# calavera/patrol

Hardware: AMD Instinct MI355X
Metric: bucket-state merges/sec + achieved HBM GB/s at 1/2/4/8 MI355X (higher is better)
Workload: dtype f64; 1 GPU; C2 merge: 100000000 replica messages -> 10000000-bucket table (2^25 slots), Zipf(1.1); keys_per_gpu=10000000, slots_per_gpu=33554432, parallelism=shard1, name_bytes=2-8 (b<id>), world_size=1, full=False, exchange=False, batches_in_hbm=28

## Files before the change

### patrol_amd/csrc/phip_engine.hip

```cpp
#include <sys/random.h>

#include <chrono>
#include <cstdlib>
#include <cstring>
#include <hip/hip_runtime.h>
#include <rocprim/rocprim.hpp>

#include <algorithm>
#include <cstdarg>
#include <cstdio>
#include <cstring>
#include <mutex>
#include <string>
#include <vector>

#include "patrolhip.h"
#include "phip_kernels.hpp"
#include "phip_host.hpp"

using namespace phip;

namespace {

#ifndef PHIP_SORT_BITS
// ... 617 lines not shown
  out->cap = shard_cap(units, per_unit);
  if ((rc = ensure(h, base_id, (size_t)kShards * out->cap, &out->base)) ||
      (rc = ensure(h, B_MSCNT, 2 * kShards, &out->cnt)))
    return rc;
  if (zero) HIPCHK(h, hipMemsetAsync(out->cnt, 0, kShards * sizeof(u32), h->stream));
  return PHIP_OK;
}

int pack_sharded(phip_handle* h, const Sharded& sh, u32 total_slot, u32* out, u32* total) {
  k_shard_scan<<<1, kShards, 0, h->stream>>>(sh.cnt, h->ctr, total_slot, nullptr, 0, nullptr,
                                             nullptr, nullptr);
  HIPCHK(h, hipGetLastError());
  int rc;
  if ((rc = read_ctr(h))) return rc;
  *total = h->ctr_host[total_slot];
  if (*total) {
    Launch l(h, "k_shard_compact");
    dim3 grid(grid_for(h->ctr_host[kCtrShardMax]), kShards);
    k_shard_compact<<<grid, 256, 0, h->stream>>>(sh.base, sh.cap, sh.cnt, out);
    HIPCHK(h, hipGetLastError());
  }
  return PHIP_OK;
}


enum class PassAsk { kPolicy, kMayUndo, kIsolate, kNoIsolate };

template <class In>
PassKind pass_kind(const phip_handle* h, PassAsk ask) {
  if (ask == PassAsk::kIsolate) return PassKind::kIsolating;
  if (ask == PassAsk::kNoIsolate) return PassKind::kClassified;
  if (h->iso_always || h->iso_left > 0) return PassKind::kIsolating;
  if (ask == PassAsk::kMayUndo && In::kSoa && !h->classify_first && h->opt_left == 0)
    return PassKind::kOptimistic;
  return PassKind::kClassified;
}

inline size_t undo_counts(const phip_handle* h) { return (size_t)h->ncu * kFastPerCU * (kFastBlock / 64); }

struct UndoLayout {
  u32 grid, waves, cap;
  u64 halves;
};
inline UndoLayout undo_layout(u32 n, u32 ncu) {
  UndoLayout l;
  l.grid = fast_grid_on(ncu, n);
  l.waves = l.grid * (kFastBlock / 64);
  l.cap = undo_wave_cap(n, l.grid);
  l.halves = (u64)l.waves * l.cap * 2;
  return l;
}

inline u32* fctr(phip_handle* h, u32 par) { return h->ctr + kCtrWords * (1 + par); }

inline u32* fast_counts(phip_handle* h, u32 par) {
  return (u32*)h->buf[B_FSCNT].p + par * 2 * kShards;
}

int dirty_set(phip_handle* h, DirtySet* d, u32** dlist) {
  int rc;
  u64* b;
  if ((rc = ensure(h, B_DTAB, DirtySet::kWords, &b)) || (rc = ensure(h, B_DLIST, kDirtyCap, dlist)))
    return rc;
  *d = DirtySet::at(b);
  return PHIP_OK;
}
struct SubBatch {
  uint64_t *off, *a, *t;
  int64_t* e;
  u8* len;
  u32* map;
};
int sub_batch(phip_handle* h, SubBatch* b) {
  constexpr size_t m = kSubBatchCap;
  int rc;
  if ((rc = ensure(h, B_SOFF, m, &b->off)) || (rc = ensure(h, B_SLEN, m, &b->len)) ||
      (rc = ensure(h, B_SA, m, &b->a)) || (rc = ensure(h, B_ST, m, &b->t)) ||
      (rc = ensure(h, B_SE, m, &b->e)) || (rc = ensure(h, B_SMAP, m, &b->map)))
    return rc;
  return PHIP_OK;
}

int fast_shards(phip_handle* h, u32 n, u32 par, Sharded* out) {
  int rc;
  u32* c;
  out->cap = shard_cap((n + 63) / 64, 64);
  if ((rc = ensure(h, B_MSHARD, (size_t)kShards * out->cap, &out->base)) ||
      (rc = ensure(h, B_FSCNT, 4 * kShards, &c)))
    return rc;
  out->cnt = fast_counts(h, par);
  return PHIP_OK;
}

template <class Src>
int fork_hot(phip_handle* h, Src src, FastPass* p) {
  if (p->n < kHotMinBatch) return PHIP_OK;
  HIPCHK(h, hipStreamWaitEvent(h->stream2, h->ev_fork, 0));
  int rc;
  if ((rc = build_hot(h, src, p->n, h->stream2, nullptr, p))) return rc;
  HIPCHK(h, hipEventRecord(h->ev_join, h->stream2));
  p->hot_join = true;
  return PHIP_OK;
}

bool keep_take(phip_handle* h, FastPass* p);
template <class HotSrc>
// ... 63 lines not shown
  p->c = fctr(h, p->par);
  ++h->nfast;
  if (reset) {
    k_batch_reset<<<1, kShards, 0, h->stream>>>(p->c, fast_counts(h, p->par));
    HIPCHK(h, hipGetLastError());
  }
  if (p->kind == PassKind::kOptimistic) return front_optimistic(h, hsrc, status, p);
  h->keep.agree = false;
  return front_classified(h, in, hsrc, status, p);
}

inline bool holds(const phip_handle* h, BufId id, size_t bytes) {
  return h->buf[id].cap >= std::max<size_t>(bytes, 64) + 64;
}
inline bool back_fits(const phip_handle* h, u32 n) {
  return holds(h, B_MISS, (size_t)n * sizeof(u32)) &&
         holds(h, B_MSHARD, (size_t)kShards * shard_cap((n + 63) / 64, 64) * sizeof(u32)) &&
         holds(h, B_FSCNT, 4 * kShards * sizeof(u32)) &&
         holds(h, B_ULOG, (size_t)undo_layout(n, (u32)h->ncu).halves * sizeof(u64x2));
}

template <class In>
int fast_back(phip_handle* h, In in, FastPass& p, bool queued) {
  const u32 n = p.n;
  const bool iso = p.kind == PassKind::kIsolating;
  u32* miss;
  int rc;
  Sharded msh;
  DirtySet dset{};
  SubBatch sb{};
  u32* dlist = nullptr;
  if ((rc = ensure(h, B_MISS, n, &miss)) || (rc = fast_shards(h, n, p.par, &msh))) return rc;
  if (iso) {
    if ((rc = dirty_set(h, &dset, &dlist)) || (rc = sub_batch(h, &sb))) return rc;
    Launch l(h, "k_dirty_build");
    k_dirty_build<In><<<1, 1024, 0, h->stream>>>(in, n, p.c, dlist, dset, table(h));
    HIPCHK(h, hipGetLastError());
  }
  if (p.hot_join) HIPCHK(h, hipStreamWaitEvent(h->stream, h->ev_join, 0));
  switch (p.kind) {
    case PassKind::kOptimistic:
      if constexpr (In::kSoa) {
        const UndoLayout ul = undo_layout(n, (u32)h->ncu);
        p.log.cap = ul.cap;
        if ((rc = ensure(h, B_ULOG, (size_t)ul.halves, &p.log.base))) return rc;
        u8* kstatus = PHIP_STATUS_IN_KERNEL ? p.fill : nullptr;
        if (p.fill && !kstatus) HIPCHK(h, hipMemsetAsync(p.fill, PHIP_ST_MERGED, n, h->stream));
        Launch l(h, "k_receive_fast");
        auto* kern = p.hot_nw == 2   ? k_receive_fast<In, true, 2>
                     : p.hot_nw == 3 ? k_receive_fast<In, true, 3>
                                     : k_receive_fast<In, true, 0>;
        kern<<<ul.grid, kFastBlock, 0, h->stream>>>(
            in, 0, n, table(h), msh, p.c, p.hot, p.dir, nullptr, nullptr, p.log,
            (uint4*)p.hot_zero, p.hot_age != 0, p.gate, kstatus);
      }
      break;
    case PassKind::kClassified:
    case PassKind::kIsolating: {
      Launch l(h, "k_receive_fast");
      k_receive_fast<In><<<fast_grid(h, n), kFastBlock, 0, h->stream>>>(
          in, 0, n, table(h), msh, p.c, p.hot, p.dir, iso ? dset.key : nullptr, p.mark,
          UndoLog{}, (uint4*)p.hot_zero, 0u, nullptr, nullptr);
    }
  }
  HIPCHK(h, hipGetLastError());
  if (p.hot_zero) h->hot_clean = p.hot_zero;
  if (iso) {
    {
      Launch l(h, "k_dirty_pass");
      const unsigned g = (unsigned)std::max<u64>(
          1, std::min<u64>(((u64)n + 1023) / 1024, (u64)h->ncu * 2));
      k_dirty_pass<In><<<g, 1024, 0, h->stream>>>(in, n, p.c, p.mark, dset.key, table(h), msh);
      HIPCHK(h, hipGetLastError());
    }
    k_batch_end<In><<<1, kShards, 0, h->stream>>>(
        in, p.c, dset.key, table(h),
        SubOut{sb.off, sb.len, sb.a, sb.t, sb.e, sb.map, kSubBatchCap}, msh.cnt,
        h->ctr_map + kCtrWords * (1 + p.par), kCtrWords,
        queued ? fast_counts(h, p.par ^ 1u) : nullptr, fctr(h, p.par ^ 1u));
  } else {
    k_shard_scan<<<1, kShards, 0, h->stream>>>(msh.cnt, p.c, kCtrMiss,
                                               h->ctr_map + kCtrWords * (1 + p.par), kCtrWords,
                                               queued ? fast_counts(h, p.par ^ 1u) : nullptr,
                                               fctr(h, p.par ^ 1u), p.gate);
  }
  HIPCHK(h, hipGetLastError());
  HIPCHK(h, hipEventRecord(h->ev_ctr[p.par], h->stream));
  if (!queued) HIPCHK(h, hipEventSynchronize(h->ev_ctr[p.par]));
  return PHIP_OK;
}

constexpr u32 kIsoKeep = 256;
constexpr u32 kOptBackoff = 256;

constexpr u32 kHotKeepPasses = 32;
bool keep_take(phip_handle* h, FastPass* p) {
  phip_handle::HotKeep& k = h->keep;
  if (p->n < kHotMinBatch || !k.have || !k.agree || k.sagged || k.served >= kHotKeepPasses ||
      k.gen != h->layout_gen || k.base != h->buf[B_HOT].p)
    return false;
  p->hot = (const HotHdr*)((u8*)k.base + kHotSlotsAt + k.slot * kHotSlotBytes);
  p->dir = (const HotEntry*)(p->hot + 1);
  p->hot_age = k.served++;
  p->hot_nw = k.maxlen <= kShortName ? 2u : k.maxlen <= kInlineName ? 3u : 0u;
  return true;
}
bool keep_sagged(const phip_handle* h, const FastPass& p, const u32* c) {
  const phip_handle::HotKeep& k = h->keep;
  return p.hot_age != 0 && (unsigned __int128)c[kCtrHotHits] * k.ref_n * 8 <
                               (unsigned __int128)k.ref_hits * p.n * 7;
}
void keep_collect(phip_handle* h, const FastPass& p, const u32* c) {
  phip_handle::HotKeep& k = h->keep;
  if (p.kind != PassKind::kOptimistic) {
    k.agree = false;
    return;
  }
  if (p.built) {
    k.agree = c[kCtrHotOwn] > 0 && (u64)c[kCtrHotKept] * 8 >= (u64)c[kCtrHotOwn] * 7;
    k.maxlen = c[kCtrHotMaxLen];
    k.ref_hits = c[kCtrHotHits];
    k.ref_n = p.n;
    k.sagged = false;
  } else if (keep_sagged(h, p, c)) {
    k.sagged = true;
  }
}

inline const u32* fmirror(const phip_handle* h, u32 par) { return h->ctr_host + kCtrWords * (1 + par); }

bool apply_policy(phip_handle* h, const FastPass& p) {
  const u32* c = fmirror(h, p.par);
  if (p.kind == PassKind::kOptimistic) {
// ... 1348 lines not shown
  *out = nullptr;
  if (cfg->log2_slots < 4 || cfg->log2_slots > 31) return PHIP_ERR_INVALID;
  int ndev = 0;
  if (hipGetDeviceCount(&ndev) != hipSuccess || ndev == 0) return PHIP_ERR_NO_DEVICE;
  if (cfg->device < 0 || cfg->device >= ndev) return PHIP_ERR_NO_DEVICE;
  phip_handle* h = new phip_handle;
  h->device = cfg->device;
  h->L = h->L_open = cfg->log2_slots;
  h->cap = 1ull << h->L;
  h->load_pct = cfg->max_load_pct ? std::min<u32>(cfg->max_load_pct, 95) : 90;
  h->max_load = load_limit(h->cap, h->load_pct);
  h->grow = !(cfg->flags & PHIP_CFG_NO_GROW);
  h->iso_always = cfg->flags & PHIP_CFG_ISOLATE;
  h->classify_first = cfg->flags & PHIP_CFG_CLASSIFY_FIRST;
  h->small = !(cfg->flags & PHIP_CFG_NO_SMALL);
  h->track = cfg->flags & PHIP_CFG_TRACK_CHANGES;
  h->arena_cap = h->arena_open = cfg->arena_bytes ? cfg->arena_bytes : (1ull << 20);
  if (cfg->debug_tag_bits && cfg->debug_tag_bits < 64) h->tag_mask = (1ull << cfg->debug_tag_bits) - 1;
  if (cfg->flags & PHIP_CFG_FIXED_SEED) {
    h->seed = cfg->hash_seed;
  } else if (getrandom(&h->seed, sizeof h->seed, 0) != (ssize_t)sizeof h->seed) {
    h->seed = seeded_mix((u64)std::chrono::steady_clock::now().time_since_epoch().count(),
                         (u64)(uintptr_t)h);
  }
  auto fail = [&](hipError_t e) {
    phip_close(h);
    (void)e;
    return PHIP_ERR_HIP;
  };
  hipError_t e;
  if ((e = hipSetDevice(h->device)) != hipSuccess) return fail(e);
  if ((e = hipDeviceGetAttribute(&h->ncu, hipDeviceAttributeMultiprocessorCount, h->device)) !=
      hipSuccess)
    return fail(e);
  if ((e = hipStreamCreateWithFlags(&h->own_stream, hipStreamNonBlocking)) != hipSuccess)
    return fail(e);
  h->stream = h->own_stream;
  if ((e = hipStreamCreateWithFlags(&h->stream2, hipStreamNonBlocking)) != hipSuccess) return fail(e);
  if ((e = hipStreamCreateWithFlags(&h->stream3, hipStreamNonBlocking)) != hipSuccess) return fail(e);
  if ((e = hipEventCreateWithFlags(&h->ev_fork, hipEventDisableTiming)) != hipSuccess) return fail(e);
  if ((e = hipEventCreateWithFlags(&h->ev_join, hipEventDisableTiming)) != hipSuccess) return fail(e);
  if ((e = hipEventCreateWithFlags(&h->ev_fork3, hipEventDisableTiming)) != hipSuccess) return fail(e);
  if ((e = hipEventCreateWithFlags(&h->ev_join3, hipEventDisableTiming)) != hipSuccess) return fail(e);
  if ((e = hipEventCreateWithFlags(&h->ev_gather, hipEventDisableTiming)) != hipSuccess) return fail(e);
  if ((e = hipEventCreateWithFlags(&h->ev_gather3, hipEventDisableTiming)) != hipSuccess)
    return fail(e);
  if ((e = hipEventCreateWithFlags(&h->ev_pack, hipEventDisableTiming)) != hipSuccess) return fail(e);
  for (hipEvent_t& ev : h->ev_ctr)
    if ((e = hipEventCreateWithFlags(&ev, hipEventDisableTiming)) != hipSuccess) return fail(e);
  if ((e = hipMalloc(&h->recs, h->cap * sizeof(Rec))) != hipSuccess) return fail(e);
  if ((e = hipMalloc(&h->aux, h->cap * sizeof(u32))) != hipSuccess) return fail(e);
  if ((e = hipMalloc(&h->arena, h->arena_cap + 64)) != hipSuccess) return fail(e);
  if ((e = hipMalloc(&h->arena_cursor, 64)) != hipSuccess) return fail(e);
  if ((e = hipMalloc(&h->ctr, 3 * kCtrWords * sizeof(u32))) != hipSuccess) return fail(e);
  if ((e = hipHostMalloc(&h->ctr_host, 3 * kCtrWords * sizeof(u32),
                         hipHostMallocMapped | hipHostMallocCoherent)) != hipSuccess ||
      (e = hipHostGetDevicePointer((void**)&h->ctr_map, h->ctr_host, 0)) != hipSuccess)
    return fail(e);
  if ((e = hipMemsetAsync(h->recs, 0, h->cap * sizeof(Rec), h->stream)) != hipSuccess) return fail(e);
  if ((e = hipMemsetAsync(h->aux, 0, h->cap * sizeof(u32), h->stream)) != hipSuccess) return fail(e);
  if (h->track && alloc_marks(h, h->cap, &h->marks)) return fail(hipErrorOutOfMemory);
  if ((e = hipMemsetAsync(h->arena_cursor, 0, 64, h->stream)) != hipSuccess) return fail(e);
  if ((e = hipMemsetAsync(h->ctr, 0, 3 * kCtrWords * sizeof(u32), h->stream)) != hipSuccess)
    return fail(e);
  if ((e = hipStreamSynchronize(h->stream)) != hipSuccess) return fail(e);
  *out = h;
  return PHIP_OK;
}

void phip_close(phip_handle* h) {
  if (!h) return;
  (void)hipSetDevice(h->device);
  if (h->pend.active) (void)after_error(h, finish_pending(h));
  if (h->stream) (void)hipStreamSynchronize(h->stream);
  if (h->stream2) (void)hipStreamSynchronize(h->stream2);
  if (h->stream3) (void)hipStreamSynchronize(h->stream3);
  if (h->stream4) (void)hipStreamSynchronize(h->stream4);
  for (auto& b : h->buf)
    if (b.p) (void)hipFree(b.p);
  for (auto& t : h->event_pool) {
    (void)hipEventDestroy(t.a);
    (void)hipEventDestroy(t.b);
  }
  if (h->recs) (void)hipFree(h->recs);
  if (h->aux) (void)hipFree(h->aux);
  if (h->marks.state) (void)hipFree(h->marks.state);
  if (h->arena) (void)hipFree(h->arena);
  if (h->arena_cursor) (void)hipFree(h->arena_cursor);
  if (h->ctr) (void)hipFree(h->ctr);
  if (h->ctr_host) (void)hipHostFree(h->ctr_host);
  if (h->small_pin) (void)hipHostFree(h->small_pin);
  if (h->ev_fork) (void)hipEventDestroy(h->ev_fork);
  if (h->ev_join) (void)hipEventDestroy(h->ev_join);
  if (h->ev_fork3) (void)hipEventDestroy(h->ev_fork3);
  if (h->ev_join3) (void)hipEventDestroy(h->ev_join3);
  if (h->ev_gather) (void)hipEventDestroy(h->ev_gather);
  if (h->ev_gather3) (void)hipEventDestroy(h->ev_gather3);
  if (h->ev_pack) (void)hipEventDestroy(h->ev_pack);
  for (hipEvent_t ev : h->ev_ctr)
    if (ev) (void)hipEventDestroy(ev);
  if (h->stream2) (void)hipStreamDestroy(h->stream2);
  if (h->stream3) (void)hipStreamDestroy(h->stream3);
  if (h->stream4) (void)hipStreamDestroy(h->stream4);
  if (h->ev_t4a) (void)hipEventDestroy(h->ev_t4a);
  if (h->ev_t4b) (void)hipEventDestroy(h->ev_t4b);
  if (h->own_stream) {
    (void)hipStreamSynchronize(h->own_stream);
    (void)hipStreamDestroy(h->own_stream);
  }
  delete h;
}

const char* phip_last_error(const phip_handle* h) { return h ? h->err.c_str() : "null handle"; }

int phip_flush(phip_handle* h) {
  if (!h) return PHIP_ERR_INVALID;
// ... 1908 lines not shown
```

### patrol_amd/csrc/phip_kernels.hpp

```cpp
#pragma once
#include <type_traits>

#include "phip_device.hpp"

namespace phip {

constexpr int kBlock = 256;

template <bool NT, class T>
__device__ inline T ld(const T* p) {
  if constexpr (NT) return __builtin_nontemporal_load(p);
  else return *p;
}

__device__ inline u64 load_be64(const u8* p) {
  u64 v = 0;
#pragma unroll
  for (int k = 0; k < 8; ++k) v = (v << 8) | p[k];
  return v;
}

struct NamesOffs {
  const u8* blob;
  const u32* offs;
// ... 173 lines not shown
constexpr u32 kCtrHotExt = 23;
constexpr u32 kCtrHotMaxLen = 24;
constexpr u32 kCtrGateShut = 22;
constexpr u32 kCtrEgIncast = kCtrHotExt;
constexpr u32 kCtrEgN = kCtrHotMaxLen;
constexpr u32 kCtrEgErr = 25;
constexpr u32 kCtrEgIncastBytes = 26;
constexpr u32 kCtrEgBytes = 28;
constexpr u32 kCtrChgMarks = 30;
constexpr u32 kCtrChgCleared = 31;
constexpr u32 kCtrWords = 32;
__host__ __device__ constexpr u32 ctr_reset_value(u32 w) {
  return (w == kCtrStop || w == kCtrDirty) ? ~0u : 0u;
}
static_assert(kCtrNDirty < kCtrResetWords && kCtrBadName < kCtrResetWords &&
                  kCtrOccupied < kCtrResetWords && kCtrStop < kCtrResetWords &&
                  kCtrLogOver < kCtrResetWords && kCtrLogCount < kCtrResetWords &&
                  kCtrArenaFull < kCtrResetWords && kCtrTableFull < kCtrResetWords &&
                  kCtrHotHits < kCtrResetWords && kCtrDirty < kCtrResetWords,
              "the words kernels accumulate into from the batch's reset value");
static_assert(kCtrTableFull == kCtrArenaFull + 1, "evict_idle clears both flags in one memset");
static_assert(kCtrLongBytes % 2 == 0 && kCtrLongBytes >= kCtrResetWords &&
              kCtrLongBytes + 2 <= kCtrWords, "an aligned u64 outside the reset");
static_assert(kCtrNDefer >= kCtrResetWords && kCtrNDefer < kCtrWords &&
              kCtrNSorted >= kCtrResetWords && kCtrNSorted < kCtrWords &&
              kCtrHotOwn >= kCtrResetWords && kCtrHotKept < kCtrWords &&
              kCtrGateShut >= kCtrResetWords && kCtrGateShut < kCtrWords, "outside the reset");
static_assert(kCtrEgIncast > kCtrGateShut && kCtrEgErr < kCtrEgIncastBytes &&
              kCtrEgIncastBytes % 2 == 0 && kCtrEgBytes == kCtrEgIncastBytes + 2 &&
              kCtrEgBytes + 2 <= kCtrWords, "the egress words: two aligned u64 behind three u32");
static_assert(kCtrChgMarks == kCtrEgBytes + 2 && kCtrChgCleared == kCtrChgMarks + 1 &&
              kCtrChgCleared < kCtrWords, "the change set's words: zeroed in one memset");

__host__ __device__ inline bool gate_shut(const u32* c) {
  return c[kCtrDirty] != ~0u || c[kCtrStop] != ~0u || c[kCtrNDirty] != 0 || c[kCtrLogOver] != 0 ||
         c[kCtrMiss] != 0 || c[kCtrTableFull] != 0;
}
static_assert(kCtrResetWords <= kShards && kCtrWords <= kShards,
              "k_batch_reset and shard_scan's host mirror: one lane per word");

__global__ __launch_bounds__(kShards) void k_batch_reset(u32* ctr, u32* shard_cnt) {
  const u32 t = threadIdx.x;
  if (t < kCtrResetWords) ctr[t] = ctr_reset_value(t);
  if (shard_cnt) shard_cnt[t] = 0;
}

__device__ inline void shard_scan(u32* cnt, u32* ctr, u32 tot, u32* host, u32 words, u32* next,
                                  u32* next_ctr, const u32* gate = nullptr);
__global__ __launch_bounds__(kShards) void k_shard_scan(u32* cnt, u32* ctr, u32 tot, u32* host,
                                                        u32 words, u32* next, u32* next_ctr,
                                                        const u32* gate) {
  shard_scan(cnt, ctr, tot, host, words, next, next_ctr, gate);
}
__device__ inline void shard_scan(u32* cnt, u32* ctr, u32 tot, u32* host, u32 words, u32* next,
                                  u32* next_ctr, const u32* gate) {
  __shared__ u32 v[kShards];
  __shared__ u32 wmax[kShards / 64];
  if (gate && gate_shut(gate)) next = nullptr;
  const u32 t = threadIdx.x, c = cnt[t];
  v[t] = c;
  u32 m = c;
  for (u32 d = 32; d; d >>= 1) m = max(m, (u32)__shfl_xor((int)m, d));
  if ((t & 63) == 0) wmax[t >> 6] = m;
  __syncthreads();
  for (u32 off = 1; off < kShards; off <<= 1) {
    const u32 x = t >= off ? v[t - off] : 0u;
    __syncthreads();
    v[t] += x;
    __syncthreads();
  }
  cnt[kShards + t] = v[t] - c;
  const u32 total = v[kShards - 1];
  u32 mx = 0;
  for (u32 w = 0; w < kShards / 64; ++w) mx = max(mx, wmax[w]);
  if (t == 0) {
    ctr[tot] = total;
    ctr[kCtrShardMax] = mx;
  }
  if (host && t < words) {
    const u32 w = t == tot ? total : t == kCtrShardMax ? mx : ctr[t];
    __hip_atomic_store(&host[t], w, __ATOMIC_RELAXED, __HIP_MEMORY_SCOPE_SYSTEM);
  }
  if (next) {
    if (t < kCtrResetWords) next_ctr[t] = ctr_reset_value(t);
    next[t] = 0;
  }
}

__global__ __launch_bounds__(256) void k_shard_compact(const u32* __restrict__ base, u32 cap,
                                                       const u32* __restrict__ cnt,
                                                       u32* __restrict__ out) {
  const u32 s = blockIdx.y, j = blockIdx.x * 256 + threadIdx.x;
  if (j < cnt[s]) out[cnt[kShards + s] + j] = base[(size_t)s * cap + j];
}

template <bool Co = false>
__device__ inline bool name_equal(const Rec& r, const Name& nm, const u8* src, const u8* arena) {
  const u64 r0 = r.name0 & ~0xFF00ull;
  if ((r0 & 0xFFu) != (nm.w0 & 0xFFu)) return false;
  if (nm.len <= kInlineName) return r0 == nm.w0 && r.name1 == nm.w1 && r.name2 == nm.w2;
  if (r.name1 != nm.w1 || r.name2 != nm.w2) return false;
  return long_tail_equal<Co>(arena, r.name0 >> 32, src, nm.off, nm.len);
}

enum ProbeResult : int { kFound = 0, kMiss = 1, kPending = 2, kFull = 3 };

__host__ __device__ inline u64 seeded_mix(u64 tag, u64 seed) {
  u64 x = tag ^ seed;
  x ^= x >> 33;
  x *= 0xff51afd7ed558ccdull;
  x ^= x >> 33;
  x *= 0xc4ceb9fe1a85ec53ull;
  x ^= x >> 33;
  return x;
}

struct Table {
  Rec* recs;
  u32* aux;
  const u8* arena;
  u32 L;
  u64 tag_mask;
  u64 seed;
  __device__ inline u64 tag(u64 h) const { return tag_of(h & tag_mask); }
  __device__ inline u32 home(u64 tag) const { return (u32)(seeded_mix(tag, seed) >> (64 - L)); }
  __device__ inline u32 mask() const { return (u32)((1ull << L) - 1); }
};

__device__ inline Rec load_rec(const Rec* p) {
  const uint4* q = reinterpret_cast<const uint4*>(p);
  uint4 a = q[0], b = q[1], c = q[2], d = q[3];
  Rec r;
  r.tag = ((u64)a.y << 32) | a.x;
  r.added = ((u64)a.w << 32) | a.z;
  r.taken = ((u64)b.y << 32) | b.x;
  r.elapsed = (i64)(((u64)b.w << 32) | b.z);
  r.name0 = ((u64)c.y << 32) | c.x;
  r.name1 = ((u64)c.w << 32) | c.z;
  r.created = (i64)(((u64)d.y << 32) | d.x);
// ... 883 lines not shown
  return eq;
}

constexpr u8 kMarkDirty = 0x40;

#ifndef PHIP_UNDO_NT
#define PHIP_UNDO_NT 1
#endif
#ifndef PHIP_STATUS_IN_KERNEL
#define PHIP_STATUS_IN_KERNEL 1
#endif
constexpr u32 kUndoFlushReserve = 64 * ((kHotMax + kFastBlock - 1) / kFastBlock);
struct UndoLog {
  u64x2* base = nullptr;
  u32* cnt = nullptr;
  u32 cap = 0;
};
__host__ __device__ inline u32 fast_wave_chunks(u32 n, u32 grid) {
  const u32 nchunks = (n + 63) / 64, kw = kFastBlock / 64;
  if (grid % 8 == 0) {
    const u32 per = (nchunks + 7) / 8, waves = grid / 8 * kw;
    return (per + waves - 1) / waves;
  }
  return (nchunks + grid * kw - 1) / (grid * kw);
}
constexpr u32 kUndoSlack = 24;
__host__ __device__ inline u32 undo_wave_cap(u32 n, u32 grid) {
  return fast_wave_chunks(n, grid) * 32 + kUndoSlack + kUndoFlushReserve;
}
__device__ inline u32 lane_rank(u64 m) {
  return __builtin_amdgcn_mbcnt_hi((u32)(m >> 32), __builtin_amdgcn_mbcnt_lo((u32)m, 0u));
}
__device__ inline void undo_store(u64x2* p, u32 slot, u64 a, u64 t, i64 e) {
#if PHIP_UNDO_NT
  __builtin_nontemporal_store(u64x2{(u64)slot, a}, p);
  __builtin_nontemporal_store(u64x2{t, (u64)e}, p + 1);
#else
  p[0] = u64x2{(u64)slot, a};
  p[1] = u64x2{t, (u64)e};
#endif
}

template <u32 NW>
struct HotCompact {
  static constexpr u32 kMax = NW == 2 ? kHotMaxExt : kHotMax3;
  static constexpr u32 kNameMax = NW == 2 ? kShortName : kInlineName;
  u16 hidx[kHotIdx];
  u64 hw[NW][kMax];
  u64 hmax[3][kMax];
  u32 hrec[kMax];
};
static_assert(sizeof(HotCompact<2>) == hot_compact_bytes(2, kHotMaxExt) &&
              sizeof(HotCompact<3>) == hot_compact_bytes(3, kHotMax3), "the layouts' arithmetic");
template <class In, bool Opt = false, u32 NW = 0>
__global__ __launch_bounds__(kFastBlock) __attribute__((amdgpu_waves_per_eu(8, 8))) void k_receive_fast(
    In in, u32 lo, u32 n, Table T, Sharded miss, u32* ctr,
    const HotHdr* __restrict__ hot, const HotEntry* __restrict__ hot_dir, const u64* dtab,
    u8* __restrict__ mark, UndoLog ulog, uint4* __restrict__ hot_zero, u32 hot_kept,
    const u32* gate, u8* __restrict__ status) {
  if constexpr (Opt) {
    const bool shut = gate && gate_shut(gate);
    if (blockIdx.x == 0 && threadIdx.x == 0) ctr[kCtrGateShut] = shut;
    if (shut) return;
    if (PHIP_STATUS_IN_KERNEL == 1 && status) {
      constexpr u32 b4 = PHIP_ST_MERGED * 0x01010101u;
      const u64 head = min((u64)n, (u64)(-(uintptr_t)status & 15));
      const u64 n16 = (n - head) / 16;
      uint4* body = reinterpret_cast<uint4*>(status + head);
      for (u64 k = (u64)blockIdx.x * kFastBlock + threadIdx.x; k < n16; k += (u64)gridDim.x * kFastBlock)
        body[k] = uint4{b4, b4, b4, b4};
      if (blockIdx.x == 0) {
        if (threadIdx.x < head) status[threadIdx.x] = PHIP_ST_MERGED;
        const u64 done = head + n16 * 16;
        if (done + threadIdx.x < n) status[done + threadIdx.x] = PHIP_ST_MERGED;
      }
    }
  }
  __shared__ u32 hslot[kHotLds];
  __shared__ u64 htag[kHotMax], hw0[kHotMax], hw1[kHotMax], hw2[kHotMax];
  __shared__ u32 hrec[kHotMax], haoff[kHotMax];
  __shared__ u64 htail[kHotTailWords][kHotMax];
  __shared__ u64 hmax[3][kHotMax];
  static_assert(NW == 0 || (Opt && In::kSoa && (NW == 2 || NW == 3)), "compact: optimistic, decoded");
  using Compact = HotCompact<NW ? NW : 2>;
  __shared__ Compact hc;
  static_assert(NW != 0 || sizeof(hslot) + sizeof(htag) * 4 + sizeof(hrec) * 2 + sizeof(htail) +
                                   sizeof(hmax) + 64 <= kHotLdsBudget,
                "today's layout in half a CU's LDS");
  __shared__ u32 hhits;
  __shared__ u32 hlog[2];

  if (hot_zero)
    for (u32 k = blockIdx.x * kFastBlock + threadIdx.x; k < kHotZeroBytes / sizeof(uint4);
         k += gridDim.x * kFastBlock)
      hot_zero[k] = uint4{0, 0, 0, 0};
  const u32 ndr = !Opt && dtab ? ctr[kCtrNDirty] : 0u;
  const bool iso = !Opt && ndr != 0 && ndr <= kDirtyCap;
  if constexpr (!Opt) n = min(n, iso ? ctr[kCtrStop] : min(ctr[kCtrStop], ctr[kCtrDirty]));
  if (n <= lo) return;
  const u32 nh = !hot ? 0u : NW ? min(hot->n_ext, Compact::kMax) : min(hot->n, kHotMax);
  if constexpr (NW != 0) {
    u32* const hidx32 = reinterpret_cast<u32*>(hc.hidx);
    for (u32 j = threadIdx.x; j < kHotIdx / 2; j += kFastBlock) hidx32[j] = 0;
    for (u32 j = threadIdx.x; j < Compact::kMax; j += kFastBlock) {
      hc.hmax[0][j] = 0; hc.hmax[1][j] = 0; hc.hmax[2][j] = 0;
    }
  } else {
    for (u32 j = threadIdx.x; j < kHotLds; j += kFastBlock) hslot[j] = 0;
    for (u32 j = threadIdx.x; j < kHotMax; j += kFastBlock) {
      hmax[0][j] = 0; hmax[1][j] = 0; hmax[2][j] = 0;
    }
  }
  if (threadIdx.x == 0) hhits = 0;
  if (Opt && threadIdx.x < 2) hlog[threadIdx.x] = 0;
  __syncthreads();
  if constexpr (NW != 0) {
    u32* const hidx32 = reinterpret_cast<u32*>(hc.hidx);
    for (u32 j = threadIdx.x; j < nh; j += kFastBlock) {
      const HotEntry d = hot_dir[j];
      hc.hw[0][j] = d.w0; hc.hw[1][j] = d.w1;
      if constexpr (NW == 3) hc.hw[2][j] = d.w2;
      hc.hrec[j] = d.slot;
      bool same = (u32)(d.w0 & 0xFFu) <= Compact::kNameMax && d.slot <= T.mask();
      if (same) {
        const Rec r = load_rec(&T.recs[d.slot]);
        same = r.tag == d.tag && (rec_flags(r) & kRecPublished) && (r.name0 & ~0xFF00ull) == d.w0 &&
               r.name1 == d.w1 && r.name2 == d.w2;
      }
      if (!same) continue;
      const u32 val = (j + 1) | (hot_fp(d.tag) << 11);
      for (u32 hs = hot_home_idx(d.tag);;) {
        const u32 sh = (hs & 1) * 16;
        const u32 old = __hip_atomic_load(&hidx32[hs >> 1], __ATOMIC_RELAXED, __HIP_MEMORY_SCOPE_WORKGROUP);
        if ((old >> sh) & 0xFFFFu) { hs = (hs + 1) & (kHotIdx - 1); continue; }
        if (atomicCAS(&hidx32[hs >> 1], old, old | (val << sh)) == old) break;
      }
    }
  } else
  for (u32 j = threadIdx.x; j < nh; j += kFastBlock) {
    const HotEntry d = hot_dir[j];
    htag[j] = d.tag; hw0[j] = d.w0; hw1[j] = d.w1; hw2[j] = d.w2;
    hrec[j] = d.slot | (iso && (rec_flags(T.recs[d.slot]) & kRecDirty) ? 0x80000000u : 0u);
    haoff[j] = d.aoff;
    for (u32 k = 0; k < kHotTailWords; ++k) htail[k][j] = d.tail[k];
    if (hot_kept) {
      bool same = d.slot <= T.mask();
      if (same) {
        const Rec r = load_rec(&T.recs[d.slot]);
        const bool arena = (r.name0 & 0xFFu) > kInlineName;
        same = r.tag == d.tag && (rec_flags(r) & kRecPublished) &&
               (arena ? (r.name0 & 0xFFu) : (r.name0 & ~0xFF00ull)) == d.w0 && r.name1 == d.w1 &&
               r.name2 == d.w2 && (arena ? (u32)(r.name0 >> 32) : 0u) == d.aoff;
      }
// ... 142 lines not shown
                         cur.name1 == nm.w1 && (rec_flags(cur) & kRecPublished);
        int pr = kFound;
        if (!hit) {
          if (shortname && cur.tag == 0) {
            pr = kMiss;
          } else {
            pr = probe(T, nm, in.blob(), &s, &cur);
          }
        }
        if (pr == kFound) {
          if (iso && (rec_flags(cur) & kRecDirty)) {
            mark[i] = kMarkDirty;
          } else if constexpr (Opt) {
            grows = ea > cur.added || et > cur.taken || ee > ((u64)cur.elapsed ^ kSign);
            gs = s; ga = cur.added; gt = cur.taken; ge = cur.elapsed;
          } else {
            Rec* r = &T.recs[s];
            if (ea > cur.added) atomicMax(&r->added, ea);
            if (et > cur.taken) atomicMax(&r->taken, et);
            if (ee > ((u64)cur.elapsed ^ kSign)) atomicMax(&r->elapsed, (i64)(ee ^ kSign));
          }
        } else if (iso && shortname) {
          mark[i] = kMarkDirty;
        } else {
          missed = true;
          if (pr == kFull) atomicOr(&ctr[kCtrTableFull], 1u);
        }
      }
    }
    if constexpr (Opt) {
      const u64 gm = __ballot(grows);
      if (gm) {
        if (grows) {
          const u32 pos = lcur + lane_rank(gm);
          if (pos < lcap) {
            undo_store(lbase + 2 * (size_t)pos, gs, ga, gt, ge);
            Rec* r = &T.recs[gs];
            if (ea > ga) atomicMax(&r->added, ea);
            if (et > gt) atomicMax(&r->taken, et);
            if (ee > ((u64)ge ^ kSign)) atomicMax(&r->elapsed, (i64)(ee ^ kSign));
          }
        }
        const u32 want = lcur + (u32)__popcll(gm);
        lover += want > lcap ? want - lcap : 0u;
        lcur = min(want, lcap);
      }
    }
    miss.append(chunk, missed, i);
  }
  if (hits) atomicAdd(&hhits, hits);
  __syncthreads();
  if (threadIdx.x == 0) {
    if (hhits) atomicAdd(&ctr[kCtrHotHits], hhits);
    if (blockIdx.x == 0) ctr[kCtrHotEntries] = nh;
  }

  if constexpr (NW != 0) {
    for (u32 jb = wave * 64; jb < nh; jb += kFastBlock) {
      const u32 j = jb + lane;
      bool lg = false;
      u64 xa = 0, xt = 0, xe = 0, ca = 0, ct = 0, ce = 0;
      Rec* r = nullptr;
      if (j < nh) {
        xa = hc.hmax[0][j]; xt = hc.hmax[1][j]; xe = hc.hmax[2][j];
        if (xa | xt | xe) {
          r = &T.recs[hc.hrec[j]];
          ca = r->added; ct = r->taken; ce = (u64)r->elapsed ^ kSign;
          lg = xa > ca || xt > ct || xe > ce;
        }
      }
      const u64 gm = __ballot(lg);
      const u32 pos = lcur + lane_rank(gm);
      if (lg && pos < ulog.cap) {
        undo_store(lbase + 2 * (size_t)pos, hc.hrec[j], ca, ct, (i64)(ce ^ kSign));
        if (xa > ca) atomicMax(&r->added, xa);
        if (xt > ct) atomicMax(&r->taken, xt);
        if (xe > ce) atomicMax(&r->elapsed, (i64)(xe ^ kSign));
      }
      const u32 want = lcur + (u32)__popcll(gm);
      lover += want > ulog.cap ? want - ulog.cap : 0u;
      lcur = min(want, ulog.cap);
    }
    if (lane == 0) {
      ulog.cnt[blockIdx.x * kWaves + wave] = lcur;
      if (lcur) atomicAdd(&hlog[0], lcur);
      if (lover) atomicAdd(&hlog[1], lover);
    }
    __syncthreads();
    if (threadIdx.x == 0) {
      if (hlog[0]) atomicAdd(&ctr[kCtrLogCount], hlog[0]);
      if (hlog[1]) atomicAdd(&ctr[kCtrLogOver], hlog[1]);
    }
    return;
  } else
  if constexpr (Opt) {
    for (u32 jb = wave * 64; jb < nh; jb += kFastBlock) {
      const u32 j = jb + lane;
      bool lg = false;
      u64 xa = 0, xt = 0, xe = 0, ca = 0, ct = 0, ce = 0;
      Rec* r = nullptr;
      if (j < nh) {
        xa = hmax[0][j]; xt = hmax[1][j]; xe = hmax[2][j];
        if (xa | xt | xe) {
          r = &T.recs[hrec[j] & 0x7FFFFFFFu];
          ca = r->added; ct = r->taken; ce = (u64)r->elapsed ^ kSign;
          lg = xa > ca || xt > ct || xe > ce;
        }
      }
      const u64 gm = __ballot(lg);
      if (lg) {
        undo_store(lbase + 2 * (size_t)(lcur + lane_rank(gm)), hrec[j] & 0x7FFFFFFFu, ca, ct,
                   (i64)(ce ^ kSign));
        if (xa > ca) atomicMax(&r->added, xa);
        if (xt > ct) atomicMax(&r->taken, xt);
        if (xe > ce) atomicMax(&r->elapsed, (i64)(xe ^ kSign));
      }
      lcur += (u32)__popcll(gm);
    }
    if (lane == 0) {
      ulog.cnt[blockIdx.x * kWaves + wave] = lcur;
      if (lcur) atomicAdd(&hlog[0], lcur);
      if (lover) atomicAdd(&hlog[1], lover);
    }
    __syncthreads();
    if (threadIdx.x == 0) {
      if (hlog[0]) atomicAdd(&ctr[kCtrLogCount], hlog[0]);
      if (hlog[1]) atomicAdd(&ctr[kCtrLogOver], hlog[1]);
    }
    return;
  }
  if constexpr (!Opt)
  for (u32 j = threadIdx.x; j < nh; j += kFastBlock) {
    const u64 xa = hmax[0][j], xt = hmax[1][j], xe = hmax[2][j];
    if (!(xa | xt | xe)) continue;
    Rec* r = &T.recs[hrec[j] & 0x7FFFFFFFu];
    const u64 ca = r->added, ct = r->taken, ce = (u64)r->elapsed ^ kSign;
    if (xa > ca) atomicMax(&r->added, xa);
    if (xt > ct) atomicMax(&r->taken, xt);
    if (xe > ce) atomicMax(&r->elapsed, (i64)(xe ^ kSign));
  }
}

__global__ __launch_bounds__(256) void k_undo(UndoLog L, Table T) {
  const u32 c = min(L.cnt[blockIdx.x], L.cap);
  const u64x2* p = L.base + (size_t)blockIdx.x * L.cap * 2;
  for (u32 k = threadIdx.x; k < c; k += 256) {
    const u64x2 x = p[2 * (size_t)k], y = p[2 * (size_t)k + 1];
    Rec* r = &T.recs[(u32)x.x & T.mask()];
    if (r->added > x.y) atomicMin(&r->added, x.y);
    if (r->taken > y.x) atomicMin(&r->taken, y.x);
    if (r->elapsed > (i64)y.y) atomicMin(&r->elapsed, (i64)y.y);
  }
}

constexpr u32 kCellCacheBits = 10;
constexpr u32 kCellCache = 1u << kCellCacheBits;
template <class In>
__global__ __launch_bounds__(1024) void k_dirty_pass(In in, u32 n, u32* ctr, u8* mark,
                                                     const u64* dtab, Table T, Sharded miss) {
  __shared__ u32 sidx[kDirtyCap];
  __shared__ u32 ckey[kCellCache], cmin[kCellCache];
  __shared__ u64 cmax[3][kCellCache];
  __shared__ u32 queue[16][128];
  const u32 ndr = ctr[kCtrNDirty];
  if (ndr == 0 || ndr > kDirtyCap) return;
  n = min(n, ctr[kCtrStop]);
  const DirtySet D = DirtySet::at(const_cast<u64*>(dtab));
  const u32 nv = ctr[kCtrNSorted];
  for (u32 j = threadIdx.x; j < nv; j += 1024) sidx[j] = D.idx[j];
  for (u32 j = threadIdx.x; j < kCellCache; j += 1024) {
    ckey[j] = 0; cmin[j] = ~0u;
    cmax[0][j] = 0; cmax[1][j] = 0; cmax[2][j] = 0;
  }
  __syncthreads();
  auto process = [&](u32 i) {
    u64 off, w0, w1, w2, ra, rt;
    u32 len;
    i64 re;
    const typename In::Pre p = in.pre(i);
    in.load(i, p, off, len, w0, w1, w2, ra, rt, re);
    Name nm;
// ... 4714 lines not shown
```

Baseline: 54.62 billion merges/s.

## Fuse shard scan into optimistic receive kernel via last-block ticket

The optimistic pass no longer launches a separate single-block k_shard_scan. The last block to finish k_receive_fast, chosen by an atomic ticket counter, performs the shard prefix scan, publishes counters to the host and resets the next pass's counters, reusing dead LDS as scratch. The status fill also moves to after the hot-table merge work. This removes a kernel launch and its dependency gap on the critical path, at the cost of an extra counter word, device-scope fences and coherent stores, and a serial tail in the last block.

Result: no change. 54.52 billion merges/s (-0.2%).

```diff
diff --git a/patrol_amd/csrc/phip_engine.hip b/patrol_amd/csrc/phip_engine.hip
--- a/patrol_amd/csrc/phip_engine.hip
+++ b/patrol_amd/csrc/phip_engine.hip
@@ -693,6 +693,7 @@
 }
 
 inline u32* fctr(phip_handle* h, u32 par) { return h->ctr + kCtrWords * (1 + par); }
+inline u32* fast_ticket(phip_handle* h) { return h->ctr + kCtrWords * 3; }
 
 inline u32* fast_counts(phip_handle* h, u32 par) {
   return (u32*)h->buf[B_FSCNT].p + par * 2 * kShards;
@@ -862,7 +863,9 @@
                                      : k_receive_fast<In, true, 0>;
         kern<<<ul.grid, kFastBlock, 0, h->stream>>>(
             in, 0, n, table(h), msh, p.c, p.hot, p.dir, nullptr, nullptr, p.log,
-            (uint4*)p.hot_zero, p.hot_age != 0, p.gate, kstatus);
+            (uint4*)p.hot_zero, p.hot_age != 0, p.gate, kstatus,
+            FastEnd{fast_ticket(h), h->ctr_map + kCtrWords * (1 + p.par),
+                    queued ? fast_counts(h, p.par ^ 1u) : nullptr, fctr(h, p.par ^ 1u)});
       }
       break;
     case PassKind::kClassified:
@@ -870,7 +873,7 @@
       Launch l(h, "k_receive_fast");
       k_receive_fast<In><<<fast_grid(h, n), kFastBlock, 0, h->stream>>>(
           in, 0, n, table(h), msh, p.c, p.hot, p.dir, iso ? dset.key : nullptr, p.mark,
-          UndoLog{}, (uint4*)p.hot_zero, 0u, nullptr, nullptr);
+          UndoLog{}, (uint4*)p.hot_zero, 0u, nullptr, nullptr, FastEnd{});
     }
   }
   HIPCHK(h, hipGetLastError());
@@ -888,7 +891,7 @@
         SubOut{sb.off, sb.len, sb.a, sb.t, sb.e, sb.map, kSubBatchCap}, msh.cnt,
         h->ctr_map + kCtrWords * (1 + p.par), kCtrWords,
         queued ? fast_counts(h, p.par ^ 1u) : nullptr, fctr(h, p.par ^ 1u));
-  } else {
+  } else if (p.kind != PassKind::kOptimistic) {
     k_shard_scan<<<1, kShards, 0, h->stream>>>(msh.cnt, p.c, kCtrMiss,
                                                h->ctr_map + kCtrWords * (1 + p.par), kCtrWords,
                                                queued ? fast_counts(h, p.par ^ 1u) : nullptr,
@@ -2343,7 +2346,7 @@
   if ((e = hipMalloc(&h->aux, h->cap * sizeof(u32))) != hipSuccess) return fail(e);
   if ((e = hipMalloc(&h->arena, h->arena_cap + 64)) != hipSuccess) return fail(e);
   if ((e = hipMalloc(&h->arena_cursor, 64)) != hipSuccess) return fail(e);
-  if ((e = hipMalloc(&h->ctr, 3 * kCtrWords * sizeof(u32))) != hipSuccess) return fail(e);
+  if ((e = hipMalloc(&h->ctr, 4 * kCtrWords * sizeof(u32))) != hipSuccess) return fail(e);
   if ((e = hipHostMalloc(&h->ctr_host, 3 * kCtrWords * sizeof(u32),
                          hipHostMallocMapped | hipHostMallocCoherent)) != hipSuccess ||
       (e = hipHostGetDevicePointer((void**)&h->ctr_map, h->ctr_host, 0)) != hipSuccess)
@@ -2352,7 +2355,7 @@
   if ((e = hipMemsetAsync(h->aux, 0, h->cap * sizeof(u32), h->stream)) != hipSuccess) return fail(e);
   if (h->track && alloc_marks(h, h->cap, &h->marks)) return fail(hipErrorOutOfMemory);
   if ((e = hipMemsetAsync(h->arena_cursor, 0, 64, h->stream)) != hipSuccess) return fail(e);
-  if ((e = hipMemsetAsync(h->ctr, 0, 3 * kCtrWords * sizeof(u32), h->stream)) != hipSuccess)
+  if ((e = hipMemsetAsync(h->ctr, 0, 4 * kCtrWords * sizeof(u32), h->stream)) != hipSuccess)
     return fail(e);
   if ((e = hipStreamSynchronize(h->stream)) != hipSuccess) return fail(e);
   *out = h;
diff --git a/patrol_amd/csrc/phip_kernels.hpp b/patrol_amd/csrc/phip_kernels.hpp
--- a/patrol_amd/csrc/phip_kernels.hpp
+++ b/patrol_amd/csrc/phip_kernels.hpp
@@ -249,23 +249,31 @@
                                                         const u32* gate) {
   shard_scan(cnt, ctr, tot, host, words, next, next_ctr, gate);
 }
-__device__ inline void shard_scan(u32* cnt, u32* ctr, u32 tot, u32* host, u32 words, u32* next,
-                                  u32* next_ctr, const u32* gate) {
-  __shared__ u32 v[kShards];
-  __shared__ u32 wmax[kShards / 64];
+constexpr u32 kShardScanWords = kShards + kShards / 64;
+template <bool Co>
+__device__ inline void shard_scan_at(u32* v, u32* cnt, u32* ctr, u32 tot, u32* host, u32 words,
+                                     u32* next, u32* next_ctr, const u32* gate) {
+  u32* const wmax = v + kShards;
   if (gate && gate_shut(gate)) next = nullptr;
-  const u32 t = threadIdx.x, c = cnt[t];
-  v[t] = c;
+  const u32 t = threadIdx.x;
+  const bool on = t < kShards;
+  const u32 c = !on ? 0u : Co ? __hip_atomic_load(&cnt[t], __ATOMIC_RELAXED, __HIP_MEMORY_SCOPE_AGENT) : cnt[t];
+  u32 own = 0;
+  if (Co && host && t < words) own = __hip_atomic_load(&ctr[t], __ATOMIC_RELAXED, __HIP_MEMORY_SCOPE_AGENT);
   u32 m = c;
   for (u32 d = 32; d; d >>= 1) m = max(m, (u32)__shfl_xor((int)m, d));
-  if ((t & 63) == 0) wmax[t >> 6] = m;
+  if (on) {
+    v[t] = c;
+    if ((t & 63) == 0) wmax[t >> 6] = m;
+  }
   __syncthreads();
   for (u32 off = 1; off < kShards; off <<= 1) {
-    const u32 x = t >= off ? v[t - off] : 0u;
+    const u32 x = on && t >= off ? v[t - off] : 0u;
     __syncthreads();
-    v[t] += x;
+    if (on) v[t] += x;
     __syncthreads();
   }
+  if (!on) return;
   cnt[kShards + t] = v[t] - c;
   const u32 total = v[kShards - 1];
   u32 mx = 0;
@@ -275,13 +283,19 @@
     ctr[kCtrShardMax] = mx;
   }
   if (host && t < words) {
-    const u32 w = t == tot ? total : t == kCtrShardMax ? mx : ctr[t];
+    if (!Co) own = ctr[t];
+    const u32 w = t == tot ? total : t == kCtrShardMax ? mx : own;
     __hip_atomic_store(&host[t], w, __ATOMIC_RELAXED, __HIP_MEMORY_SCOPE_SYSTEM);
   }
   if (next) {
     if (t < kCtrResetWords) next_ctr[t] = ctr_reset_value(t);
     next[t] = 0;
   }
+}
+__device__ inline void shard_scan(u32* cnt, u32* ctr, u32 tot, u32* host, u32 words, u32* next,
+                                  u32* next_ctr, const u32* gate) {
+  __shared__ u32 v[kShardScanWords];
+  shard_scan_at<false>(v, cnt, ctr, tot, host, words, next, next_ctr, gate);
 }
 
 __global__ __launch_bounds__(256) void k_shard_compact(const u32* __restrict__ base, u32 cap,
@@ -1271,30 +1285,51 @@
 };
 static_assert(sizeof(HotCompact<2>) == hot_compact_bytes(2, kHotMaxExt) &&
               sizeof(HotCompact<3>) == hot_compact_bytes(3, kHotMax3), "the layouts' arithmetic");
+__device__ inline void fast_fill_status(u8* __restrict__ status, u32 n) {
+  if (!status) return;
+  constexpr u32 b4 = PHIP_ST_MERGED * 0x01010101u;
+  const u64 head = min((u64)n, (u64)(-(uintptr_t)status & 15));
+  const u64 n16 = (n - head) / 16;
+  uint4* body = reinterpret_cast<uint4*>(status + head);
+  for (u64 k = (u64)blockIdx.x * kFastBlock + threadIdx.x; k < n16; k += (u64)gridDim.x * kFastBlock)
+    body[k] = uint4{b4, b4, b4, b4};
+  if (blockIdx.x == 0) {
+    if (threadIdx.x < head) status[threadIdx.x] = PHIP_ST_MERGED;
+    const u64 done = head + n16 * 16;
+    if (done + threadIdx.x < n) status[done + threadIdx.x] = PHIP_ST_MERGED;
+  }
+}
+struct FastEnd {
+  u32* ticket = nullptr;
+  u32* host = nullptr;
+  u32* next = nullptr;
+  u32* next_ctr = nullptr;
+};
+__device__ inline void fast_end(const FastEnd& fe, u32* lds, u32* flag, const Sharded& miss, u32* ctr,
+                                bool shut) {
+  asm volatile("s_waitcnt vmcnt(0)" ::: "memory");
+  __syncthreads();
+  if (threadIdx.x == 0) {
+    const u32 t = __hip_atomic_fetch_add(fe.ticket, 1u, __ATOMIC_RELAXED, __HIP_MEMORY_SCOPE_AGENT);
+    *flag = t == gridDim.x - 1;
+    if (t == gridDim.x - 1) {
+      __builtin_amdgcn_fence(__ATOMIC_ACQUIRE, "agent");
+      asm volatile("s_waitcnt vmcnt(0)" ::: "memory");
+    }
+  }
+  __syncthreads();
+  if (!*flag) return;
+  shard_scan_at<true>(lds, miss.cnt, ctr, kCtrMiss, fe.host, kCtrWords, shut ? nullptr : fe.next,
+                      fe.next_ctr, nullptr);
+  if (threadIdx.x == 0) st_co32(fe.ticket, 0u);
+}
+
 template <class In, bool Opt = false, u32 NW = 0>
 __global__ __launch_bounds__(kFastBlock) __attribute__((amdgpu_waves_per_eu(8, 8))) void k_receive_fast(
     In in, u32 lo, u32 n, Table T, Sharded miss, u32* ctr,
     const HotHdr* __restrict__ hot, const HotEntry* __restrict__ hot_dir, const u64* dtab,
     u8* __restrict__ mark, UndoLog ulog, uint4* __restrict__ hot_zero, u32 hot_kept,
-    const u32* gate, u8* __restrict__ status) {
-  if constexpr (Opt) {
-    const bool shut = gate && gate_shut(gate);
-    if (blockIdx.x == 0 && threadIdx.x == 0) ctr[kCtrGateShut] = shut;
-    if (shut) return;
-    if (PHIP_STATUS_IN_KERNEL == 1 && status) {
-      constexpr u32 b4 = PHIP_ST_MERGED * 0x01010101u;
-      const u64 head = min((u64)n, (u64)(-(uintptr_t)status & 15));
-      const u64 n16 = (n - head) / 16;
-      uint4* body = reinterpret_cast<uint4*>(status + head);
-      for (u64 k = (u64)blockIdx.x * kFastBlock + threadIdx.x; k < n16; k += (u64)gridDim.x * kFastBlock)
-        body[k] = uint4{b4, b4, b4, b4};
-      if (blockIdx.x == 0) {
-        if (threadIdx.x < head) status[threadIdx.x] = PHIP_ST_MERGED;
-        const u64 done = head + n16 * 16;
-        if (done + threadIdx.x < n) status[done + threadIdx.x] = PHIP_ST_MERGED;
-      }
-    }
-  }
+    const u32* gate, u8* __restrict__ status, FastEnd fe) {
   __shared__ u32 hslot[kHotLds];
   __shared__ u64 htag[kHotMax], hw0[kHotMax], hw1[kHotMax], hw2[kHotMax];
   __shared__ u32 hrec[kHotMax], haoff[kHotMax];
@@ -1308,7 +1343,21 @@
                 "today's layout in half a CU's LDS");
   __shared__ u32 hhits;
   __shared__ u32 hlog[2];
-
+  __shared__ u32 hlast;
+  static_assert(sizeof(hslot) >= kShardScanWords * sizeof(u32) &&
+                sizeof(hc.hidx) >= kShardScanWords * sizeof(u32), "the scan's scratch in the dead index");
+  u32* end_lds;
+  if constexpr (NW != 0) end_lds = reinterpret_cast<u32*>(hc.hidx);
+  else end_lds = hslot;
+  if constexpr (Opt) {
+    const bool shut = gate && gate_shut(gate);
+    if (blockIdx.x == 0 && threadIdx.x == 0) st_co32(&ctr[kCtrGateShut], shut);
+    if (shut) {
+      fast_end(fe, end_lds, &hlast, miss, ctr, true);
+      return;
+    }
+    if constexpr (PHIP_STATUS_IN_KERNEL == 3) fast_fill_status(status, n);
+  }
   if (hot_zero)
     for (u32 k = blockIdx.x * kFastBlock + threadIdx.x; k < kHotZeroBytes / sizeof(uint4);
          k += gridDim.x * kFastBlock)
@@ -1316,8 +1365,10 @@
   const u32 ndr = !Opt && dtab ? ctr[kCtrNDirty] : 0u;
   const bool iso = !Opt && ndr != 0 && ndr <= kDirtyCap;
   if constexpr (!Opt) n = min(n, iso ? ctr[kCtrStop] : min(ctr[kCtrStop], ctr[kCtrDirty]));
-  if (n <= lo) return;
-  const u32 nh = !hot ? 0u : NW ? min(hot->n_ext, Compact::kMax) : min(hot->n, kHotMax);
+  if constexpr (!Opt) {
+    if (n <= lo) return;
+  }
+  const u32 nh =!hot ? 0u : NW ? min(hot->n_ext, Compact::kMax) : min(hot->n, kHotMax);
   if constexpr (NW != 0) {
     u32* const hidx32 = reinterpret_cast<u32*>(hc.hidx);
     for (u32 j = threadIdx.x; j < kHotIdx / 2; j += kFastBlock) hidx32[j] = 0;
@@ -1566,7 +1617,10 @@
   __syncthreads();
   if (threadIdx.x == 0) {
     if (hhits) atomicAdd(&ctr[kCtrHotHits], hhits);
-    if (blockIdx.x == 0) ctr[kCtrHotEntries] = nh;
+    if (blockIdx.x == 0) {
+      if constexpr (Opt) st_co32(&ctr[kCtrHotEntries], nh);
+      else ctr[kCtrHotEntries] = nh;
+    }
   }
 
   if constexpr (NW != 0) {
@@ -1595,6 +1649,7 @@
       lover += want > ulog.cap ? want - ulog.cap : 0u;
       lcur = min(want, ulog.cap);
     }
+    if constexpr (PHIP_STATUS_IN_KERNEL == 1) fast_fill_status(status, n);
     if (lane == 0) {
       ulog.cnt[blockIdx.x * kWaves + wave] = lcur;
       if (lcur) atomicAdd(&hlog[0], lcur);
@@ -1605,6 +1660,7 @@
       if (hlog[0]) atomicAdd(&ctr[kCtrLogCount], hlog[0]);
       if (hlog[1]) atomicAdd(&ctr[kCtrLogOver], hlog[1]);
     }
+    fast_end(fe, end_lds, &hlast, miss, ctr, false);
     return;
   } else
   if constexpr (Opt) {
@@ -1631,6 +1687,7 @@
       }
       lcur += (u32)__popcll(gm);
     }
+    if constexpr (PHIP_STATUS_IN_KERNEL == 1) fast_fill_status(status, n);
     if (lane == 0) {
       ulog.cnt[blockIdx.x * kWaves + wave] = lcur;
       if (lcur) atomicAdd(&hlog[0], lcur);
@@ -1641,6 +1698,7 @@
       if (hlog[0]) atomicAdd(&ctr[kCtrLogCount], hlog[0]);
       if (hlog[1]) atomicAdd(&ctr[kCtrLogOver], hlog[1]);
     }
+    fast_end(fe, end_lds, &hlast, miss, ctr, false);
     return;
   }
   if constexpr (!Opt)
```
